# sirandreww/citizensassemblies-replication

Hardware: AMD Instinct MI355X
Metric: LEGACY panels/sec (node) at sf_e_110 shape; XtX MFMA util; speedup vs CPU (higher is better)
Workload: dtype int32/u64 (integer draw), fp4 MFMA -> exact int pairs; 1 GPU; sf_e_110: 1000000 LEGACY panels/GPU/step, k=110, n=1727, C=7, F=31, counts+pairs+unique; instance=sf_e_110, parallelism=panel shards x1, pipeline=draws on their own stream, 2 steps ahead of the counting

## Files before the change

### citizensassemblies-replication_amd/csrc/csa_legacy.hip

```cpp
#include <hip/hip_runtime.h>

#include <algorithm>
#include <type_traits>
#include <cstdlib>
#include <cstdarg>
#include <cstdio>
#include <cstring>
#include <string>
#include <vector>

#include "../../include/csa_legacy.h"

namespace {

thread_local std::string g_err;

int fail(int code, const char *fmt, ...) {
    char buf[512];
    va_list ap;
    va_start(ap, fmt);
    vsnprintf(buf, sizeof buf, fmt, ap);
    va_end(ap);
    g_err = buf;
    return code;
// ... 66 lines not shown
struct DrawArgs {
    const uint64_t *featmask;
    const int32_t *fmin, *fmax, *sel0, *rem0;
    const uint64_t *present0;
    const uint32_t *pmask;
    const int32_t *addr_next;
    int32_t n, F, W, Ws, k;
    uint32_t max_attempts, attempt_base;
    int32_t single;
    uint64_t seed, panel_begin, n_panels;
    uint64_t *panels;
    uint64_t *hashes;
    uint32_t *attempts;
    int32_t *picks;
    uint16_t *picks16;
    uint32_t *status;
    unsigned long long *stats;
    const uint64_t *panel_list;
    const unsigned long long *n_panels_dev;
    int32_t *sel_out, *rem_out;
    uint64_t *present_out;
    uint32_t *xt;
    int32_t npad;
};


template <int CTRL, int ROW_MASK = 0xF, bool BOUND_ZERO = false>
__device__ __forceinline__ int dpp(int old, int v) {
    return __builtin_amdgcn_update_dpp(old, v, CTRL, ROW_MASK, 0xF, BOUND_ZERO);
}

template <int LVL>
__device__ __forceinline__ int partner(int v) {
    if constexpr (LVL == 0) return dpp<0xB1, 0xF, true>(0, v);
    else if constexpr (LVL == 1) return dpp<0x4E, 0xF, true>(0, v);
    else if constexpr (LVL == 2) return dpp<0x141, 0xF, true>(0, v);
    else if constexpr (LVL == 3) return dpp<0x140, 0xF, true>(0, v);
    else if constexpr (LVL == 4) return __shfl_xor(v, 16);
    else return __shfl_xor(v, 32);
}

template <int LVL>
__device__ __forceinline__ uint64_t partner64(uint64_t v) {
    const uint32_t lo = (uint32_t)partner<LVL>((int)(uint32_t)v);
    const uint32_t hi = (uint32_t)partner<LVL>((int)(uint32_t)(v >> 32));
    return ((uint64_t)hi << 32) | lo;
// ... 371 lines not shown
    uint32_t k4, k2, k1;
    uint32_t r4, r2, r1;
};
__device__ __forceinline__ XtLane xt_lane_consts(int lane) {
    XtLane c;
    const bool b3 = (lane >> 3) & 1, b2 = (lane >> 2) & 1, b1 = (lane >> 1) & 1, b0 = lane & 1;
    c.s8_send = b3 ? 0x06040200u : 0x07050301u;
    c.s8_lo = b3 ? 0x03050104u : 0x05020400u;
    c.s8_hi = b3 ? 0x03070106u : 0x07020600u;
    c.k4 = b2 ? 0xF0F0F0F0u : 0x0F0F0F0Fu;
    c.k2 = b1 ? 0xCCCCCCCCu : 0x33333333u;
    c.k1 = b0 ? 0xAAAAAAAAu : 0x55555555u;
    c.r4 = b2 ? 4u : 28u;
    c.r2 = b1 ? 2u : 30u;
    c.r1 = b0 ? 1u : 31u;
    return c;
}
template <int CTRL>
__device__ __forceinline__ uint32_t xt_dpp(uint32_t v) {
    return (uint32_t)__builtin_amdgcn_update_dpp(0, (int)v, CTRL, 0xF, 0xF, true);
}
__device__ __forceinline__ uint32_t xt_merge(uint32_t x, uint32_t y, uint32_t keep, uint32_t rot) {
    const uint32_t t = __builtin_amdgcn_alignbit(y, y, rot);
    return (keep & x) | (~keep & t);
}
__device__ __forceinline__ void wave_transpose64(uint32_t &lo, uint32_t &hi, const XtLane &c) {
    {
        const auto r = __builtin_amdgcn_permlane32_swap(lo, hi, false, false);
        lo = r[0];
        hi = r[1];
    }
    {
        const uint32_t A = __builtin_amdgcn_perm(hi, lo, 0x05040100u), B = __builtin_amdgcn_perm(hi, lo, 0x07060302u);
        const auto r = __builtin_amdgcn_permlane16_swap(A, B, false, false);
        lo = __builtin_amdgcn_perm(r[1], r[0], 0x05040100u);
        hi = __builtin_amdgcn_perm(r[1], r[0], 0x07060302u);
    }
    {
        const uint32_t R = xt_dpp<0x128>(__builtin_amdgcn_perm(hi, lo, c.s8_send));
        lo = __builtin_amdgcn_perm(R, lo, c.s8_lo);
        hi = __builtin_amdgcn_perm(R, hi, c.s8_hi);
    }
    lo = xt_merge(lo, xt_dpp<0x141>(xt_dpp<0x1B>(lo)), c.k4, c.r4);
    hi = xt_merge(hi, xt_dpp<0x141>(xt_dpp<0x1B>(hi)), c.k4, c.r4);
    lo = xt_merge(lo, xt_dpp<0x4E>(lo), c.k2, c.r2);
    hi = xt_merge(hi, xt_dpp<0x4E>(hi), c.k2, c.r2);
    lo = xt_merge(lo, xt_dpp<0xB1>(lo), c.k1, c.r1);
// ... 926 lines not shown
                atomicAdd(&over_s, 1u);
        }
    }
    __syncthreads();
    for (int b = threadIdx.x; b < (int)n_bins; b += blockDim.x)
        if (h[b]) atomicAdd(hist + b, (unsigned long long)h[b]);
    if (threadIdx.x == 0 && over_s) atomicAdd(overflow, (unsigned long long)over_s);
}

}

void csa_set_last_error(const char *msg) { g_err = msg ? msg : ""; }

struct csa_instance {
    int32_t n = 0, C = 0, F = 0, W = 0, Ws = 0;
    int device = 0;
    std::vector<int32_t> pf, fmin, fmax, fcat, pool;
    std::vector<int32_t> sel0;
    std::vector<uint64_t> featmask;
    uint64_t *d_featmask = nullptr;
    int32_t *d_fmin = nullptr, *d_fmax = nullptr, *d_sel0 = nullptr, *d_rem0 = nullptr;
    uint64_t *d_present0 = nullptr;
    uint32_t *d_pmask = nullptr;
    int32_t *d_addr_next = nullptr;
    int32_t max_abs = 0;
    bool zero_max_min = false;
    bool sel_over_max = false;
    int32_t max_slack = 0;
    bool need8 = true;
    void *scratch[32] = {};
    size_t scratch_bytes[32] = {};
    hipStream_t stream = nullptr;
    hipStream_t sdraw = nullptr, spost = nullptr;
    hipEvent_t drawn = nullptr;
    uint16_t *d_picks16 = nullptr;
    size_t picks_bytes = 0;
    hipEvent_t picks_done = nullptr;
    bool picks_pending = false;
    std::vector<int32_t> rem0h, addr_h;
    std::vector<uint64_t> present0h;
    uint64_t gen = 1;
    std::vector<csa_instance *> replicas;
    std::vector<uint64_t> replica_gen;
    unsigned long long *d_stats = nullptr;
    uint64_t panels_drawn = 0;
};
// ... 152 lines not shown
        case 4: return draw_fn<G, FPL, 4, GEN>();
        case 8: if constexpr (G == 16) return draw_fn<G, FPL, 8, GEN>(); else return nullptr;
        case 16: if constexpr (G == 16) return draw_fn<G, FPL, 16, GEN>(); else return nullptr;
        default: return nullptr;
    }
}

template <int G, bool GEN>
const void *draw_fn_fw(int fpl, int wpl) {
    switch (fpl) {
        case 1: return draw_fn_w<G, 1, GEN>(wpl);
        case 2: return draw_fn_w<G, 2, GEN>(wpl);
        case 4: return draw_fn_w<G, 4, GEN>(wpl);
        default: return nullptr;
    }
}

int pow2_ceil_int(int x) {
    int p = 1;
    while (p < x) p <<= 1;
    return p;
}

int pick_draw_config(const csa_instance *I, bool general, DrawConfig &c) {
    general = general || I->d_addr_next;
    const bool reg_ok = I->F <= 32 && I->d_pmask && !I->zero_max_min && I->W <= 32 && I->max_abs < 32768 &&
                        !I->sel_over_max && I->max_slack <= 255;
    const bool lane_ok = reg_ok && I->F > 16;
    const bool wide_ok = I->F <= 64 && I->W <= 128 && !I->zero_max_min && I->max_abs < 32768 && !I->sel_over_max;
    const bool g16_ok = I->F <= 64 && I->W <= 256;
    const bool solo_ok = reg_ok && I->F <= 16;
    int choice = general ? 64 : solo_ok ? 1 : lane_ok ? 2 : wide_ok ? 8 : g16_ok ? 16 : 64;
    if (const char *e = getenv("CSA_DRAW_KERNEL")) {
        if (!general && !strcmp(e, "solo") && solo_ok) choice = 1;
        else if (!general && !strcmp(e, "lane") && lane_ok && !solo_ok) choice = 2;
        else if (!general && !strcmp(e, "wide") && wide_ok) choice = 8;
        else if (!general && !strcmp(e, "16") && g16_ok) choice = 16;
        else if (!general && !strcmp(e, "64")) choice = 64;
    }
    c.G = choice;
    if (choice == 1) {
        c.solo = true;
        c.FPL = std::max(8, pow2_ceil_int(I->F));
        c.WPL = I->W <= 4 ? 4 : I->W <= 8 ? 8 : I->W <= 16 ? 16 : I->W <= 28 ? 28 : 32;
        c.k8 = I->need8;
        c.np = c.FPL >= 16 ? slack_planes(I->max_slack) : 8;
        c.fn = solo_fn(c.FPL, c.WPL, c.k8, c.np);
        if (!c.fn) return fail(CSA_E_UNSUPPORTED, "no solo draw kernel for F=%d W=%d", I->F, I->W);
        return CSA_OK;
    }
    if (choice == 8) {
        const int fpl = (I->F + 7) / 8;
        c.wide = true;
        c.FPL = fpl <= 2 ? 2 : fpl <= 4 ? 4 : fpl <= 5 ? 5 : 8;
        c.WPL = I->W <= 32 ? 4 : I->W <= 64 ? 8 : 16;
        c.fn = wide_fn(c.FPL, c.WPL);
        if (!c.fn) return fail(CSA_E_UNSUPPORTED, "no wide draw kernel for F=%d W=%d", I->F, I->W);
        return CSA_OK;
    }
    if (choice == 2) {
        c.lane = true;
        c.FPL = std::max(8, pow2_ceil_int(I->F));
        c.WPL = I->W <= 4 ? 4 : I->W <= 8 ? 8 : I->W <= 16 ? 16 : I->W <= 28 ? 28 : 32;
        c.k8 = I->need8;
        c.np = slack_planes(I->max_slack);
        c.fn = lane_fn(c.FPL, c.WPL, c.k8, c.np);
        if (!c.fn) return fail(CSA_E_UNSUPPORTED, "no lane draw kernel for F=%d W=%d", I->F, I->W);
        return CSA_OK;
    }
    c.FPL = pow2_ceil_int((I->F + c.G - 1) / c.G);
    c.WPL = pow2_ceil_int(std::max(1, (I->W + c.G - 1) / c.G));
    if (general)
        c.fn = draw_fn_fw<64, true>(c.FPL, c.WPL);
    else
        c.fn = c.G == 16 ? draw_fn_fw<16, false>(c.FPL, c.WPL) : draw_fn_fw<64, false>(c.FPL, c.WPL);
    if (!c.fn)
        return fail(CSA_E_UNSUPPORTED, "no draw kernel for F=%d n=%d (G=%d needs FPL=%d WPL=%d)", I->F, I->n, c.G,
                    c.FPL, c.WPL);
    return CSA_OK;
}

__global__ void empty_panels_kernel(uint64_t n_panels, uint32_t *attempts, uint32_t *status, uint64_t panel_begin,
                                    int rejected) {
    const uint64_t i = (uint64_t)blockIdx.x * blockDim.x + threadIdx.x;
    if (i >= n_panels) return;
    if (rejected) {
        if (i == 0) raise_status(status, CSA_E_ATTEMPT_LIMIT, panel_begin);
    } else if (attempts) {
        attempts[i] = 1u;
    }
}

int lane_picks(csa_instance *I, uint64_t count, hipStream_t st, uint16_t **out) {
    if (!I->picks_done) HIPCHK(hipEventCreateWithFlags(&I->picks_done, hipEventDisableTiming));
    if (I->picks_pending) HIPCHK(hipStreamWaitEvent(st, I->picks_done, 0));
    const size_t bytes = std::max<uint64_t>(count, 1) * sizeof(uint16_t);
    if (I->picks_bytes < bytes) {
        if (I->picks_pending) HIPCHK(hipEventSynchronize(I->picks_done));
        if (I->d_picks16) HIPCHK(hipFree(I->d_picks16));
        I->d_picks16 = nullptr;
        I->picks_bytes = 0;
// ... 75 lines not shown
    A.W = I->W;
    A.Ws = I->Ws;
    A.k = k;
    A.max_attempts = max_attempts ? max_attempts : kDefaultMaxAttempts;
    A.attempt_base = attempt_base;
    A.single = single;
    A.seed = seed;
    A.panel_begin = panel_begin;
    A.n_panels = n_panels;
    A.panels = d_panels;
    A.hashes = d_hashes;
    A.attempts = d_attempts;
    A.picks = d_picks;
    A.picks16 = nullptr;
    A.status = d_status;
    A.stats = (single || !count_stats) ? nullptr : I->d_stats;
    A.panel_list = d_panel_list;
    A.n_panels_dev = d_list_len;
    A.sel_out = d_sel_out;
    A.rem_out = d_rem_out;
    A.present_out = d_present_out;
    A.xt = nullptr;
    A.npad = ((I->n + 255) / 256) * 256;
    if (d_picks_ext && !cfg.picks()) return fail(CSA_E_UNSUPPORTED, "this instance does not take the pick-list draw");
    csa_instance *M = const_cast<csa_instance *>(I);
    if (d_picks_ext)
        A.picks16 = d_picks_ext;
    else if (cfg.picks() && (rc = lane_picks(M, ((n_panels + 255) & ~255ull) * (uint64_t)((k + 7) & ~7), stream,
                                             &A.picks16)))
        return rc;
    const int threads = cfg.lane   ? kLaneThreads
                        : cfg.solo ? kSoloThreads
                        : cfg.wide ? kWideThreads
                                   : draw_threads(cfg.FPL, cfg.WPL);
    const int groups_wg = threads / cfg.G;
    const size_t lds = cfg.lane   ? lane_lds_bytes(cfg.FPL, cfg.WPL, I->n)
                       : cfg.solo ? solo_lds_bytes(cfg.FPL, cfg.WPL, I->n)
                       : cfg.wide ? wide_lds_bytes(cfg.G, cfg.FPL, cfg.WPL)
                                  : draw_lds_bytes(cfg.G, cfg.FPL, cfg.WPL, I->W, k, groups_wg);
    if (lds > 160 * 1024) return fail(CSA_E_UNSUPPORTED, "draw kernel needs %zu B of LDS", lds);
    static const size_t lds_pad = [] {
        const char *e = getenv("CSA_DRAW_LDS_PAD");
        return e ? (size_t)strtoull(e, nullptr, 10) : (size_t)0;
    }();
    const size_t lds_launch = (cfg.lane || cfg.solo || cfg.wide) && lds + lds_pad <= 160 * 1024 ? lds + lds_pad : lds;
    const uint64_t want = (n_panels + groups_wg - 1) / groups_wg;
// ... 228 lines not shown
    if ((rc = dalloc(&I->d_featmask, I->featmask.size())) || (rc = dalloc(&I->d_fmin, F)) ||
        (rc = dalloc(&I->d_fmax, F)) || (rc = dalloc(&I->d_sel0, F)) || (rc = dalloc(&I->d_rem0, F)) ||
        (rc = dalloc(&I->d_present0, I->W)) || (F <= 32 && (rc = dalloc(&I->d_pmask, n))) ||
        (rc = dalloc(&I->d_stats, 2))) {
        csa_instance_destroy(I);
        return rc;
    }
    std::vector<uint32_t> pmask(F <= 32 ? n : 0, 0u);
    for (int p = 0; p < (int)pmask.size(); ++p)
        for (int c = 0; c < C; ++c) pmask[p] |= 1u << person_feat[(size_t)p * C + c];
    hipError_t e = hipSuccess;
    e = e ? e : hipMemcpy(I->d_featmask, I->featmask.data(), I->featmask.size() * 8, hipMemcpyHostToDevice);
    e = e ? e : hipMemcpy(I->d_fmin, fmin, F * 4, hipMemcpyHostToDevice);
    e = e ? e : hipMemcpy(I->d_fmax, fmax, F * 4, hipMemcpyHostToDevice);
    e = e ? e : hipMemcpy(I->d_sel0, zeros.data(), F * 4, hipMemcpyHostToDevice);
    e = e ? e : hipMemcpy(I->d_rem0, I->pool.data(), F * 4, hipMemcpyHostToDevice);
    if (I->W) e = e ? e : hipMemcpy(I->d_present0, present.data(), I->W * 8, hipMemcpyHostToDevice);
    if (!pmask.empty()) e = e ? e : hipMemcpy(I->d_pmask, pmask.data(), pmask.size() * 4, hipMemcpyHostToDevice);
    e = e ? e : hipMemset(I->d_stats, 0, 16);
    if (e != hipSuccess) {
        csa_instance_destroy(I);
        return fail(CSA_E_HIP, "instance upload: %s", hipGetErrorString(e));
    }
    *out = I;
    return CSA_OK;
}

void csa_instance_destroy(csa_instance *I) {
    if (!I) return;
    ScopedDevice sd(I->device);
    if (I->picks_done && I->picks_pending) (void)hipEventSynchronize(I->picks_done);
    if (I->sdraw) (void)hipStreamSynchronize(I->sdraw);
    if (I->spost) (void)hipStreamSynchronize(I->spost);
    if (I->stream) (void)hipStreamSynchronize(I->stream);
    if (I->d_featmask) (void)hipFree(I->d_featmask);
    if (I->d_fmin) (void)hipFree(I->d_fmin);
    if (I->d_fmax) (void)hipFree(I->d_fmax);
    if (I->d_sel0) (void)hipFree(I->d_sel0);
    if (I->d_rem0) (void)hipFree(I->d_rem0);
    if (I->d_present0) (void)hipFree(I->d_present0);
    if (I->d_pmask) (void)hipFree(I->d_pmask);
    if (I->d_addr_next) (void)hipFree(I->d_addr_next);
    if (I->d_picks16) (void)hipFree(I->d_picks16);
    if (I->d_stats) (void)hipFree(I->d_stats);
    for (int i = 0; i < kScratchSlots; ++i)
        if (I->scratch[i]) (void)hipFree(I->scratch[i]);
    if (I->picks_done) (void)hipEventDestroy(I->picks_done);
    if (I->drawn) (void)hipEventDestroy(I->drawn);
    if (I->stream) (void)hipStreamDestroy(I->stream);
    if (I->sdraw) (void)hipStreamDestroy(I->sdraw);
    if (I->spost) (void)hipStreamDestroy(I->spost);
    for (csa_instance *R : I->replicas)
        if (R) csa_instance_destroy(R);
    delete I;
}

int csa_instance_draw_stats(csa_instance *I, int32_t reset, uint64_t *out) {
    if (!I || !out) return fail(CSA_E_INVALID, "draw_stats: bad arguments");
    uint64_t acc[3] = {0, 0, 0};
    std::vector<csa_instance *> all{I};
    for (csa_instance *R : I->replicas)
        if (R) all.push_back(R);
    for (csa_instance *X : all) {
        ScopedDevice sd(X->device);
// ... 57 lines not shown
    if (C) *C = I->C;
    if (F) *F = I->F;
    if (W) *W = I->W;
    return CSA_OK;
}

int csa_instance_set_state(csa_instance *I, const int32_t *sel, const int32_t *rem, const uint64_t *present) {
    if (!I) return fail(CSA_E_INVALID, "null instance");
    ScopedDevice sd(I->device);
    std::vector<int32_t> zeros(I->F, 0);
    std::vector<uint64_t> all(I->W, 0ull);
    for (int p = 0; p < I->n; ++p) all[p >> 6] |= 1ull << (p & 63);
    int32_t mx = 0;
    for (int f = 0; f < I->F; ++f) mx = std::max(mx, std::abs(I->fmin[f]));
    I->sel_over_max = false;
    I->max_slack = 0;
    for (int f = 0; f < I->F; ++f) {
        const int32_t s = sel ? sel[f] : 0;
        if (sel) mx = std::max(mx, std::abs(s));
        if (s > I->fmax[f] || (I->fmax[f] > 0 && s == I->fmax[f])) I->sel_over_max = true;
        if (I->fmax[f] > 0) I->max_slack = std::max(I->max_slack, I->fmax[f] - s);
    }
    I->max_abs = mx;
    update_need8(I);
    if (present)
        for (int w = 0; w < I->W; ++w)
            if (present[w] & ~all[w]) return fail(CSA_E_INVALID, "present mask has bits beyond n");
    HIPCHK(hipMemcpy(I->d_sel0, sel ? sel : zeros.data(), I->F * 4, hipMemcpyHostToDevice));
    I->sel0.assign(sel ? sel : zeros.data(), (sel ? sel : zeros.data()) + I->F);
    HIPCHK(hipMemcpy(I->d_rem0, rem ? rem : I->pool.data(), I->F * 4, hipMemcpyHostToDevice));
    if (I->W) HIPCHK(hipMemcpy(I->d_present0, present ? present : all.data(), I->W * 8, hipMemcpyHostToDevice));
    if (rem) I->rem0h.assign(rem, rem + I->F); else I->rem0h.clear();
    if (present) I->present0h.assign(present, present + I->W); else I->present0h.clear();
    ++I->gen;
    return CSA_OK;
}

int csa_instance_set_address(csa_instance *I, const int32_t *addr_next) {
    if (!I) return fail(CSA_E_INVALID, "null instance");
    ScopedDevice sd(I->device);
    if (I->picks_pending) HIPCHK(hipEventSynchronize(I->picks_done));
    if (!addr_next) {
        if (I->d_addr_next) HIPCHK(hipFree(I->d_addr_next));
        I->d_addr_next = nullptr;
        I->addr_h.clear();
        ++I->gen;
        return CSA_OK;
    }
    for (int p = 0; p < I->n; ++p)
        if (addr_next[p] < 0 || addr_next[p] >= I->n) return fail(CSA_E_INVALID, "addr_next[%d] out of range", p);
    if (!I->d_addr_next) {
        int rc = dalloc(&I->d_addr_next, (size_t)I->n);
        if (rc) return rc;
    }
    HIPCHK(hipMemcpy(I->d_addr_next, addr_next, (size_t)I->n * 4, hipMemcpyHostToDevice));
    I->addr_h.assign(addr_next, addr_next + I->n);
    ++I->gen;
    return CSA_OK;
// ... 918 lines not shown
```

### citizensassemblies-replication_amd/csrc/draw_lane.inc

```

constexpr int kLaneThreads = 256;
constexpr int kLaneSlots = 8;

__host__ __device__ inline size_t lane_lds_bytes(int FN, int WN, int n) {
    const size_t LS = (size_t)WN + 1;
    const size_t draw = (size_t)2 * FN * LS * 8 + 64
                        + (size_t)((n + 3) & ~3) * 4
                        + (size_t)4 * FN * 4
                        + (size_t)2 * WN * 8
                        + (size_t)(kLaneThreads / 64) * kLaneSlots * WN * 8
                        + (size_t)(kLaneThreads / 64) * kLaneSlots * FN * 4;
    const size_t pack = (size_t)(kLaneThreads / 2) * (2 * (size_t)WN + 1) * 4;
    return draw > pack ? draw : pack;
}

__device__ __forceinline__ void philox_lane(uint32_t &c0, uint32_t &c1, uint32_t &c2, uint32_t &c3, uint32_t k0,
                                            uint32_t k1) {
#pragma unroll
    for (int r = 0; r < 10; ++r) {
        if (r) {
            k0 += 0x9E3779B9u;
            k1 += 0xBB67AE85u;
        }
        asm volatile("" : "+s"(k0), "+s"(k1));
// ... 10 lines not shown
    int r;
    asm("v_bcnt_u32_b32 %0, %1, %2" : "=v"(r) : "v"(x), "v"(acc));
    return r;
}

typedef short short2_t __attribute__((ext_vector_type(2)));
__device__ __forceinline__ short2_t as_s2(int v) { return __builtin_bit_cast(short2_t, v); }
__device__ __forceinline__ int as_i(short2_t v) { return __builtin_bit_cast(int, v); }
__device__ __forceinline__ int kneed(int key) { return (int)as_s2(key).x; }
__device__ __forceinline__ int krem(int key) { return (int)as_s2(key).y; }
__device__ __forceinline__ int kpack(int need, int rem) { return (int)(((uint32_t)rem << 16) | ((uint32_t)need & 0xFFFFu)); }
__device__ __forceinline__ bool kbeats(int key, int best) {
    const short2_t a = as_s2(key), b = as_s2(best);
    return (int)a.x * (int)b.y > (int)b.x * (int)a.y;
}

#ifndef CSA_LANE_OCC
#define CSA_LANE_OCC 4
#endif

typedef signed char schar4_t __attribute__((ext_vector_type(4)));
__device__ __forceinline__ int k8need(int key) { return (int)__builtin_bit_cast(schar4_t, key).x; }
__device__ __forceinline__ int k8rem(int key) { return (int)as_s2(key).y; }
__device__ __forceinline__ int k8pack(int need, int rem, int idx) {
    return (int)(((uint32_t)rem << 16) | ((uint32_t)(idx + 1 - (need < 0)) & 0xFFu) << 8 | ((uint32_t)need & 0xFFu));
}
__device__ __forceinline__ int k8idx1(int key) { return (int)((((uint32_t)key >> 8) & 0xFFu) + (((uint32_t)key >> 7) & 1u)); }
template <bool K8>
constexpr int kDrawSentinel = K8 ? (1 << 16) | 0x009C : (1 << 16) | 0xFF9C;
__device__ __forceinline__ bool k8beats(int key, int best) {
    return k8need(key) * k8rem(best) > k8need(best) * k8rem(key);
}

#ifdef CSA_LANE_STAMPS
__device__ unsigned long long g_lane_stamps[24];
#define LANE_STAMP(k)                                              \
    do {                                                           \
        const uint64_t t_ = __builtin_amdgcn_s_memtime();          \
        st_acc[k] += t_ - st_prev;                                 \
        st_prev = t_;                                              \
    } while (0)
#define LANE_REGION(name, k, cond)                                                                \
    do {                                                                                          \
        __builtin_amdgcn_sched_barrier(0);       \
        asm volatile(";@region " #name);                                                          \
        const uint64_t b_ = __ballot(cond);                                                       \
         \
                                   \
        atomicAdd(&st_cnt[k], (uint32_t)(b_ != 0ull &&                                            \
                                         (int)(threadIdx.x & 63) == __ffsll((long long)__ballot(1)) - 1)); \
    } while (0)
#else
#define LANE_STAMP(k) \
    do {              \
    } while (0)
#define LANE_REGION(name, k, cond) \
    do {                           \
    } while (0)
#endif


constexpr int kPackRows = 128;
template <int PPW, int CH>
__device__ __forceinline__ void pack_tile_rows(const DrawArgs &A, uint32_t *tile, uint64_t pb, int rows) {
    static_assert(CH == 4 || CH == 8, "8- or 16-byte chunks");
    using unit_t = typename std::conditional<CH == 8, uint4, uint2>::type;
    const int W = A.W, k = A.k, kpad = (k + 7) & ~7, nch = kpad / CH;
    __syncthreads();
    const int R = 2 * W + 1;
    for (int t = threadIdx.x; 4 * t < kPackRows * R; t += blockDim.x) {
        if (4 * t + 3 < kPackRows * R) *reinterpret_cast<uint4 *>(tile + 4 * t) = make_uint4(0u, 0u, 0u, 0u);
        else for (int u = 4 * t; u < kPackRows * R; ++u) tile[u] = 0u;
    }
    const uint64_t wg = pb / PPW;
    const int p0 = (int)(pb % PPW);
    const unit_t *src = reinterpret_cast<const unit_t *>(A.picks16 + (wg * nch * PPW + p0) * CH);
    const int nu = nch * kPackRows;
    __syncthreads();
    constexpr int kChunks = 8;
    for (int e0 = 0; e0 < nu; e0 += kChunks * kLaneThreads) {
        unit_t v[kChunks];
#pragma unroll
        for (int u = 0; u < kChunks; ++u) {
            const int e = e0 + u * kLaneThreads + (int)threadIdx.x;
            const int r = e & (kPackRows - 1), c = e >> 7;
            if (e < nu && r < rows) v[u] = src[(uint64_t)c * PPW + r];
        }
#pragma unroll
        for (int u = 0; u < kChunks; ++u) {
            const int e = e0 + u * kLaneThreads + (int)threadIdx.x;
            const int r = e & (kPackRows - 1), c = e >> 7;
            if (e < nu && r < rows) {
                uint32_t w4[4];
                if constexpr (CH == 8) {
                    w4[0] = v[u].x; w4[1] = v[u].y; w4[2] = v[u].z; w4[3] = v[u].w;
                } else {
                    w4[0] = v[u].x; w4[1] = v[u].y; w4[2] = w4[3] = 0u;
                }
#pragma unroll
                for (int h = 0; h < CH; ++h) {
                    if (c * CH + h < k) {
                        const uint32_t q = (h & 1) ? w4[h >> 1] >> 16 : w4[h >> 1] & 0xFFFFu;
                        atomicOr(&tile[r * R + (q >> 5)], 1u << (q & 31));
                    }
                }
            }
        }
    }
    __syncthreads();
    uint64_t *dst = A.panels + pb * (uint64_t)W;
    const float rw = 1.0f / (float)W;
    for (int t = threadIdx.x; t < rows * W; t += blockDim.x) {
        const int r = min(rows - 1, (int)(((float)t + 0.5f) * rw)), w = t - r * W;
        dst[t] = (uint64_t)tile[r * R + 2 * w] | ((uint64_t)tile[r * R + 2 * w + 1] << 32);
    }
    if (A.hashes) {
        const int r = threadIdx.x >> 1, sub = threadIdx.x & 1;
        uint64_t h1 = 0, h2 = 0;
        if (r < rows)
            for (int w = sub; w < W; w += 2) {
                const uint64_t x = (uint64_t)tile[r * R + 2 * w] | ((uint64_t)tile[r * R + 2 * w + 1] << 32);
                h1 += fmix_a(x ^ ((uint64_t)w * 0x9E3779B97F4A7C15ull));
                h2 += fmix_b(x + ((uint64_t)w + 1) * 0xD6E8FEB86659FD93ull);
            }
        h1 += partner64<0>(h1);
        h2 += partner64<0>(h2);
        if (r < rows && sub == 0) {
            A.hashes[2 * (pb + r)] = h1;
            A.hashes[2 * (pb + r) + 1] = h2;
        }
    }
}

template <int NWAVES>
__device__ __forceinline__ void emit_xt_rows(const DrawArgs &A, const uint32_t *tile, uint64_t pb, int rows, int lane,
                                             int wave) {
    const XtLane tc = xt_lane_consts(lane);
    const int W = A.W, R = 2 * W + 1, nwd = A.npad / 64, nb = (rows + 63) / 64;
    const uint64_t b0 = pb / 64;
    for (int e = wave; e < nb * nwd; e += NWAVES) {
        const int blk = e / nwd, w = e - blk * nwd, r = 64 * blk + lane;
        uint32_t lo = 0u, hi = 0u;
        if (w < W && r < rows) {
            lo = tile[r * R + 2 * w];
            hi = tile[r * R + 2 * w + 1];
        }
        wave_transpose64(lo, hi, tc);
        uint32_t *x32 = A.xt + 2 * (b0 + blk) * (uint64_t)A.npad + 64 * w + lane;
        x32[0] = lo;
        x32[A.npad] = hi;
    }
}

template <int FN, int WN, int SK, int NP, bool K8>
__global__ __launch_bounds__(kLaneThreads, CSA_LANE_OCC) void draw_lane_kernel(DrawArgs A) {
    constexpr int G = 2;
    constexpr int LS = WN + 1;
    constexpr int WS = (WN + 1) / 2;
    constexpr int FPL = FN / G, WPL = WN / G;
    static_assert(FN == 32 && WN <= 32 && (WN % 2) == 0 && SK >= 1 && NP >= 1 && NP <= 8, "lane draw layout");
    extern __shared__ uint64_t smem[];
    const int F = A.F, W = A.W, n = A.n, k = A.k;
    uint64_t *fm = smem;
    uint64_t *fm_rev = fm + FN * LS + 8;
    uint32_t *pm = reinterpret_cast<uint32_t *>(fm_rev + FN * LS);
    int32_t *need0_s = reinterpret_cast<int32_t *>(pm + ((n + 3) & ~3));
    int32_t *rem0_s = need0_s + FN, *mnx_s = need0_s + 2 * FN;
    uint64_t *pres0_s = reinterpret_cast<uint64_t *>(need0_s + 4 * FN);
    uint64_t *pres0_rev = pres0_s + WN;
    uint64_t *slot_all = pres0_s + 2 * WN;
    int32_t *dec_all = reinterpret_cast<int32_t *>(slot_all + (kLaneThreads / 64) * kLaneSlots * WN);

    uint32_t live = 0;
    for (int f = 0; f < F; ++f) live |= (uint32_t)(A.fmax[f] != 0) << f;
    for (int t = threadIdx.x; t < FN * LS; t += blockDim.x) {
        const int f = t / LS, w = t - f * LS;
        const bool lf = f < F && ((live >> f) & 1u);
        fm[t] = (lf && w < W) ? A.featmask[f * A.Ws + w] : 0ull;
        const int wr = WN - 1 - w;
        fm_rev[t] = (lf && w < WN && wr < W) ? __brevll(A.featmask[f * A.Ws + wr]) : 0ull;
    }
    for (int t = threadIdx.x; t < n; t += blockDim.x) pm[t] = A.pmask[t] & live;
    for (int t = threadIdx.x; t < FN; t += blockDim.x) {
        const bool v = t < F && ((live >> t) & 1u);
        if constexpr (K8) {
            need0_s[t] = k8pack(v ? A.fmin[t] - A.sel0[t] : 0, v ? A.rem0[t] : 0, t);
        } else {
            need0_s[t] = v ? A.fmin[t] - A.sel0[t] : 0;
            rem0_s[t] = v ? A.rem0[t] : 0;
        }
    }
    for (int t = threadIdx.x; t < 16; t += blockDim.x) {
        const int h = t >> 3, bit = t & 7;
        uint32_t P = 0;
        for (int j = 0; j < FPL; ++j) {
            const int f = h * FPL + j;
            const bool v = f < F && ((live >> f) & 1u);
            const int sl = v ? A.fmax[f] - A.sel0[f] : 255;
            P |= (uint32_t)((sl >> bit) & 1) << j;
        }
        mnx_s[t] = (int32_t)P;
    }
    for (int t = threadIdx.x; t < WN; t += blockDim.x) {
        pres0_s[t] = t < W ? A.present0[t] : 0ull;
        pres0_rev[t] = WN - 1 - t < W ? __brevll(A.present0[WN - 1 - t]) : 0ull;
    }
    __syncthreads();

    const int lane = threadIdx.x & 63, wave = threadIdx.x >> 6;
    const int glane = lane & 1, gbase = lane & ~1;
    const int fbase = glane * FPL;
    const uint64_t *fmx = glane ? fm_rev : fm;
    const int poff = glane ? 64 * WN - 1 : 0, psgn = glane ? -1 : 1;
    uint64_t *slots = slot_all + (size_t)wave * kLaneSlots * WN;
    int32_t *decs = dec_all + wave * kLaneSlots * FN;
    const uint32_t key0 = (uint32_t)A.seed, key1 = (uint32_t)(A.seed >> 32);
    const uint64_t n_groups = (uint64_t)__builtin_amdgcn_readfirstlane(gridDim.x * (blockDim.x / G));
    const uint64_t *pres0_l = glane ? pres0_rev : pres0_s;
    uint64_t i = (uint64_t)blockIdx.x * (blockDim.x / G) + (threadIdx.x / G);
    bool active = i < A.n_panels;
    if (active && __hip_atomic_load(&A.status[0], __ATOMIC_RELAXED, __HIP_MEMORY_SCOPE_AGENT) != 0u) active = false;
    bool started = false;
    uint32_t a = 0;
    int s = 0;
    int key[FPL];
    uint64_t rm[WPL];
    uint32_t pacc_lo = 0u, pacc_hi = 0u;
    uint32_t sp[NP];
#pragma unroll
    for (int q = 0; q < NP; ++q) sp[q] = 0u;
// ... 410 lines not shown
```

### citizensassemblies-replication_amd/csrc/draw_solo.inc

```

constexpr int kSoloThreads = 256;
constexpr int kSoloSlots = 8;

__host__ __device__ inline size_t solo_lds_bytes(int FN, int WN, int n) {
    const size_t LS = (size_t)WN + 1;
    const size_t draw = (size_t)FN * LS * 8
                        + (size_t)((n + 3) & ~3) * 4
                        + (size_t)4 * FN * 4
                        + (size_t)WN * 8
                        + (size_t)(kSoloThreads / 64) * kSoloSlots * WN * 8
                        + (size_t)(kSoloThreads / 64) * kSoloSlots * FN * 4;
    const size_t pack = (size_t)kPackRows * (2 * (size_t)WN + 1) * 4;
    return draw > pack ? draw : pack;
}

#ifndef CSA_SOLO_OCC
#define CSA_SOLO_OCC 3
#endif
#ifndef CSA_SOLO_OCC8
#define CSA_SOLO_OCC8 4
#endif

template <int FN, int WN, int NP, bool K8>
__global__ __launch_bounds__(kSoloThreads, FN <= 8 ? CSA_SOLO_OCC8 : CSA_SOLO_OCC) void draw_solo_kernel(DrawArgs A) {
    constexpr int LS = WN + 1;
    constexpr bool kSlackPlanes = FN >= 16;
    static_assert(FN <= 32 && WN <= 32 && (FN % 8) == 0 && (WN % 2) == 0 && NP >= 1 && NP <= 8, "solo draw layout");
    extern __shared__ uint64_t smem[];
    const int F = A.F, W = A.W, n = A.n, k = A.k;
    uint64_t *fm = smem;
    uint32_t *pm = reinterpret_cast<uint32_t *>(fm + FN * LS);
    int32_t *need0_s = reinterpret_cast<int32_t *>(pm + ((n + 3) & ~3));
    int32_t *rem0_s = need0_s + FN, *mnx_s = need0_s + 2 * FN;
    uint64_t *pres0_s = reinterpret_cast<uint64_t *>(need0_s + 4 * FN);
    uint64_t *slot_all = pres0_s + WN;
    int32_t *cnt_all = reinterpret_cast<int32_t *>(slot_all + (kSoloThreads / 64) * kSoloSlots * WN);

    uint32_t live = 0;
    for (int f = 0; f < F; ++f) live |= (uint32_t)(A.fmax[f] != 0) << f;
    for (int t = threadIdx.x; t < FN * LS; t += blockDim.x) {
        const int f = t / LS, w = t - f * LS;
        const bool lf = f < F && ((live >> f) & 1u);
        fm[t] = (lf && w < W) ? A.featmask[f * A.Ws + w] : 0ull;
    }
    for (int t = threadIdx.x; t < n; t += blockDim.x) pm[t] = A.pmask[t] & live;
    for (int t = threadIdx.x; t < FN; t += blockDim.x) {
        const bool v = t < F && ((live >> t) & 1u);
        if constexpr (K8) {
            need0_s[t] = k8pack(v ? A.fmin[t] - A.sel0[t] : 0, v ? A.rem0[t] : 0, t);
        } else {
            need0_s[t] = v ? A.fmin[t] - A.sel0[t] : 0;
            rem0_s[t] = v ? A.rem0[t] : 0;
        }
    }
    if constexpr (!kSlackPlanes) {
        for (int t = threadIdx.x; t < FN; t += blockDim.x) {
            const bool v = t < F && ((live >> t) & 1u);
            mnx_s[t] = v ? A.fmin[t] - A.fmax[t] + 1 : -(1 << 30);
        }
    }
    for (int t = threadIdx.x; kSlackPlanes && t < 8; t += blockDim.x) {
        uint32_t P = 0;
        for (int j = 0; j < FN; ++j) {
            const bool v = j < F && ((live >> j) & 1u);
            const int sl = v ? A.fmax[j] - A.sel0[j] : 255;
            P |= (uint32_t)((sl >> t) & 1) << j;
        }
        mnx_s[t] = (int32_t)P;
    }
    for (int t = threadIdx.x; t < WN; t += blockDim.x) pres0_s[t] = t < W ? A.present0[t] : 0ull;
    __syncthreads();

    const int lane = threadIdx.x & 63, wave = threadIdx.x >> 6;
    uint64_t *slots = slot_all + (size_t)wave * kSoloSlots * WN;
    int32_t *cnts = cnt_all + wave * kSoloSlots * FN;
    const uint32_t key0 = (uint32_t)A.seed, key1 = (uint32_t)(A.seed >> 32);
    const uint64_t n_lanes = (uint64_t)__builtin_amdgcn_readfirstlane(gridDim.x * blockDim.x);
    uint64_t i = (uint64_t)blockIdx.x * blockDim.x + threadIdx.x;
    bool active = i < A.n_panels;
    if (active && __hip_atomic_load(&A.status[0], __ATOMIC_RELAXED, __HIP_MEMORY_SCOPE_AGENT) != 0u) active = false;
    bool started = false;
    uint32_t a = 0;
    int s = 0;
    int key[FN];
    uint64_t rm[WN];
    uint64_t pacc = 0ull;
    uint32_t sp[NP];
#pragma unroll
    for (int q = 0; q < NP; ++q) sp[q] = 0u;
    const int kpad = (k + 7) & ~7;
#pragma unroll
    for (int j = 0; j < FN; ++j) key[j] = 0;
#pragma unroll
    for (int j = 0; j < WN; ++j) rm[j] = 0ull;
// ... 320 lines not shown
```

Before: 284.0 million panels/s.

## Prebuild draw shared-memory image on host and copy it in with vector loads

Builds a host-side packed image of the per-instance draw tables (feature masks, reversed masks, pmask, need/rem keys, slack planes, presence) and uploads it once, so each lane/solo draw block fills shared memory with a bulk uint4 copy instead of computing the tables per block. It also restructures the pick-packing loop so each thread owns a row and skips per-element bounds checks on full chunks. The panel emit and xt transpose stores are changed to use incremental pointer arithmetic, and xt_merge now uses a bitop3 instruction. The image must be rebuilt whenever the start state changes, which adds host work and a device buffer per instance.

```diff
diff --git a/citizensassemblies-replication_amd/csrc/csa_legacy.hip b/citizensassemblies-replication_amd/csrc/csa_legacy.hip
--- a/citizensassemblies-replication_amd/csrc/csa_legacy.hip
+++ b/citizensassemblies-replication_amd/csrc/csa_legacy.hip
@@ -112,6 +112,7 @@
     uint64_t *present_out;
     uint32_t *xt;
     int32_t npad;
+    const uint64_t *image;
 };
 
 
@@ -529,7 +530,7 @@
 }
 __device__ __forceinline__ uint32_t xt_merge(uint32_t x, uint32_t y, uint32_t keep, uint32_t rot) {
     const uint32_t t = __builtin_amdgcn_alignbit(y, y, rot);
-    return (keep & x) | (~keep & t);
+    return __builtin_amdgcn_bitop3_b32(keep, x, t, 0xCA);
 }
 __device__ __forceinline__ void wave_transpose64(uint32_t &lo, uint32_t &hi, const XtLane &c) {
     {
@@ -1502,6 +1503,7 @@
     int32_t *d_fmin = nullptr, *d_fmax = nullptr, *d_sel0 = nullptr, *d_rem0 = nullptr;
     uint64_t *d_present0 = nullptr;
     uint32_t *d_pmask = nullptr;
+    uint64_t *d_image = nullptr;
     int32_t *d_addr_next = nullptr;
     int32_t max_abs = 0;
     bool zero_max_min = false;
@@ -1700,6 +1702,14 @@
     return p;
 }
 
+bool reg_kernel_shape(const csa_instance *I, bool &lane, int &fn, int &wn) {
+    if (I->F > 32 || I->W > 32 || !I->d_pmask) return false;
+    lane = I->F > 16;
+    fn = std::max(8, pow2_ceil_int(I->F));
+    wn = I->W <= 4 ? 4 : I->W <= 8 ? 8 : I->W <= 16 ? 16 : I->W <= 28 ? 28 : 32;
+    return true;
+}
+
 int pick_draw_config(const csa_instance *I, bool general, DrawConfig &c) {
     general = general || I->d_addr_next;
     const bool reg_ok = I->F <= 32 && I->d_pmask && !I->zero_max_min && I->W <= 32 && I->max_abs < 32768 &&
@@ -1719,8 +1729,8 @@
     c.G = choice;
     if (choice == 1) {
         c.solo = true;
-        c.FPL = std::max(8, pow2_ceil_int(I->F));
-        c.WPL = I->W <= 4 ? 4 : I->W <= 8 ? 8 : I->W <= 16 ? 16 : I->W <= 28 ? 28 : 32;
+        bool lane_shape;
+        reg_kernel_shape(I, lane_shape, c.FPL, c.WPL);
         c.k8 = I->need8;
         c.np = c.FPL >= 16 ? slack_planes(I->max_slack) : 8;
         c.fn = solo_fn(c.FPL, c.WPL, c.k8, c.np);
@@ -1738,8 +1748,8 @@
     }
     if (choice == 2) {
         c.lane = true;
-        c.FPL = std::max(8, pow2_ceil_int(I->F));
-        c.WPL = I->W <= 4 ? 4 : I->W <= 8 ? 8 : I->W <= 16 ? 16 : I->W <= 28 ? 28 : 32;
+        bool lane_shape;
+        reg_kernel_shape(I, lane_shape, c.FPL, c.WPL);
         c.k8 = I->need8;
         c.np = slack_planes(I->max_slack);
         c.fn = lane_fn(c.FPL, c.WPL, c.k8, c.np);
@@ -1755,6 +1765,81 @@
     if (!c.fn)
         return fail(CSA_E_UNSUPPORTED, "no draw kernel for F=%d n=%d (G=%d needs FPL=%d WPL=%d)", I->F, I->n, c.G,
                     c.FPL, c.WPL);
+    return CSA_OK;
+}
+
+int draw_image_build(csa_instance *I) {
+    bool lane = false;
+    int FN = 0, WN = 0;
+    if (!reg_kernel_shape(I, lane, FN, WN)) return CSA_OK;
+    const int F = I->F, W = I->W, n = I->n, LS = WN + 1;
+    const DrawImage L = draw_image_layout(lane, FN, WN, n);
+    std::vector<uint32_t> img((size_t)2 * L.words, 0u);
+    auto put64 = [&](int word, uint64_t v) {
+        img[2 * (size_t)word] = (uint32_t)v;
+        img[2 * (size_t)word + 1] = (uint32_t)(v >> 32);
+    };
+    auto brev64 = [](uint64_t x) {
+        uint64_t r = 0;
+        for (int b = 0; b < 64; ++b) r |= ((x >> b) & 1ull) << (63 - b);
+        return r;
+    };
+    uint32_t live = 0;
+    for (int f = 0; f < F; ++f) live |= (uint32_t)(I->fmax[f] != 0) << f;
+    auto alive = [&](int f) { return f < F && ((live >> f) & 1u); };
+    for (int f = 0; f < F; ++f) {
+        if (!alive(f)) continue;
+        const uint64_t *row = I->featmask.data() + (size_t)f * I->Ws;
+        for (int w = 0; w < W; ++w) put64(f * LS + w, row[w]);
+        for (int t = 0; lane && t < WN; ++t)
+            if (WN - 1 - t < W) put64(L.fm_rev + f * LS + t, brev64(row[WN - 1 - t]));
+    }
+    for (int p = 0; p < n; ++p) {
+        uint32_t m = 0;
+        for (int c = 0; c < I->C; ++c) m |= 1u << I->pf[(size_t)p * I->C + c];
+        img[2 * (size_t)L.pm + p] = m & live;
+    }
+    uint32_t *need0 = img.data() + 2 * (size_t)L.need0, *rem0 = need0 + FN, *mnx = need0 + 2 * FN;
+    const int32_t *rem = I->rem0h.empty() ? I->pool.data() : I->rem0h.data();
+    for (int t = 0; t < FN; ++t) {
+        const int need = alive(t) ? I->fmin[t] - I->sel0[t] : 0, rm = alive(t) ? rem[t] : 0;
+        if (I->need8) {
+            need0[t] = (uint32_t)k8pack(need, rm, t);
+        } else {
+            need0[t] = (uint32_t)need;
+            rem0[t] = (uint32_t)rm;
+        }
+    }
+    if (FN >= 16) {
+        const int halves = lane ? 2 : 1, FPL = FN / halves;
+        for (int h = 0; h < halves; ++h)
+            for (int bit = 0; bit < 8; ++bit) {
+                uint32_t P = 0;
+                for (int j = 0; j < FPL; ++j) {
+                    const int f = h * FPL + j;
+                    const int sl = alive(f) ? I->fmax[f] - I->sel0[f] : 255;
+                    P |= (uint32_t)((sl >> bit) & 1) << j;
+                }
+                mnx[8 * h + bit] = P;
+            }
+    } else {
+        for (int t = 0; t < FN; ++t) mnx[t] = (uint32_t)(alive(t) ? I->fmin[t] - I->fmax[t] + 1 : -(1 << 30));
+    }
+    for (int t = 0; t < WN; ++t) {
+        auto pres = [&](int w) -> uint64_t {
+            if (w >= W) return 0ull;
+            if (!I->present0h.empty()) return I->present0h[w];
+            return w < n / 64 ? ~0ull : (1ull << (n & 63)) - 1ull;
+        };
+        put64(L.pres0 + t, pres(t));
+        if (lane) put64(L.pres0_rev + t, brev64(pres(WN - 1 - t)));
+    }
+    ScopedDevice sd(I->device);
+    if (!I->d_image) {
+        int rc = dalloc(&I->d_image, (size_t)L.words);
+        if (rc) return rc;
+    }
+    HIPCHK(hipMemcpy(I->d_image, img.data(), (size_t)L.words * 8, hipMemcpyHostToDevice));
     return CSA_OK;
 }
 
@@ -1876,6 +1961,8 @@
     A.present_out = d_present_out;
     A.xt = nullptr;
     A.npad = ((I->n + 255) / 256) * 256;
+    A.image = I->d_image;
+    if ((cfg.lane || cfg.solo) && !A.image) return fail(CSA_E_INVALID, "the instance has no draw image");
     if (d_picks_ext && !cfg.picks()) return fail(CSA_E_UNSUPPORTED, "this instance does not take the pick-list draw");
     csa_instance *M = const_cast<csa_instance *>(I);
     if (d_picks_ext)
@@ -2150,6 +2237,10 @@
         csa_instance_destroy(I);
         return fail(CSA_E_HIP, "instance upload: %s", hipGetErrorString(e));
     }
+    if ((rc = draw_image_build(I))) {
+        csa_instance_destroy(I);
+        return rc;
+    }
     *out = I;
     return CSA_OK;
 }
@@ -2168,6 +2259,7 @@
     if (I->d_rem0) (void)hipFree(I->d_rem0);
     if (I->d_present0) (void)hipFree(I->d_present0);
     if (I->d_pmask) (void)hipFree(I->d_pmask);
+    if (I->d_image) (void)hipFree(I->d_image);
     if (I->d_addr_next) (void)hipFree(I->d_addr_next);
     if (I->d_picks16) (void)hipFree(I->d_picks16);
     if (I->d_stats) (void)hipFree(I->d_stats);
@@ -2271,18 +2363,18 @@
         if (I->fmax[f] > 0) I->max_slack = std::max(I->max_slack, I->fmax[f] - s);
     }
     I->max_abs = mx;
-    update_need8(I);
     if (present)
         for (int w = 0; w < I->W; ++w)
             if (present[w] & ~all[w]) return fail(CSA_E_INVALID, "present mask has bits beyond n");
     HIPCHK(hipMemcpy(I->d_sel0, sel ? sel : zeros.data(), I->F * 4, hipMemcpyHostToDevice));
     I->sel0.assign(sel ? sel : zeros.data(), (sel ? sel : zeros.data()) + I->F);
+    update_need8(I);
     HIPCHK(hipMemcpy(I->d_rem0, rem ? rem : I->pool.data(), I->F * 4, hipMemcpyHostToDevice));
     if (I->W) HIPCHK(hipMemcpy(I->d_present0, present ? present : all.data(), I->W * 8, hipMemcpyHostToDevice));
     if (rem) I->rem0h.assign(rem, rem + I->F); else I->rem0h.clear();
     if (present) I->present0h.assign(present, present + I->W); else I->present0h.clear();
     ++I->gen;
-    return CSA_OK;
+    return draw_image_build(I);
 }
 
 int csa_instance_set_address(csa_instance *I, const int32_t *addr_next) {
diff --git a/citizensassemblies-replication_amd/csrc/draw_lane.inc b/citizensassemblies-replication_amd/csrc/draw_lane.inc
--- a/citizensassemblies-replication_amd/csrc/draw_lane.inc
+++ b/citizensassemblies-replication_amd/csrc/draw_lane.inc
@@ -56,7 +56,7 @@
 typedef signed char schar4_t __attribute__((ext_vector_type(4)));
 __device__ __forceinline__ int k8need(int key) { return (int)__builtin_bit_cast(schar4_t, key).x; }
 __device__ __forceinline__ int k8rem(int key) { return (int)as_s2(key).y; }
-__device__ __forceinline__ int k8pack(int need, int rem, int idx) {
+__host__ __device__ inline int k8pack(int need, int rem, int idx) {
     return (int)(((uint32_t)rem << 16) | ((uint32_t)(idx + 1 - (need < 0)) & 0xFFu) << 8 | ((uint32_t)need & 0xFFu));
 }
 __device__ __forceinline__ int k8idx1(int key) { return (int)((((uint32_t)key >> 8) & 0xFFu) + (((uint32_t)key >> 7) & 1u)); }
@@ -93,6 +93,42 @@
     } while (0)
 #endif
 
+struct DrawImage {
+    int fm_rev, pm, need0, pres0, pres0_rev, words;
+};
+__host__ __device__ constexpr DrawImage draw_image_layout(bool lane, int FN, int WN, int n) {
+    DrawImage L = {};
+    L.fm_rev = FN * (WN + 1) + 8;
+    L.pm = lane ? L.fm_rev + FN * (WN + 1) : FN * (WN + 1);
+    L.need0 = L.pm + ((n + 3) & ~3) / 2;
+    L.pres0 = L.need0 + 2 * FN;
+    L.pres0_rev = L.pres0 + WN;
+    L.words = L.pres0 + (lane ? 2 : 1) * WN;
+    return L;
+}
+__device__ __forceinline__ void load_draw_image(uint64_t *smem, const uint64_t *image, int n16) {
+    constexpr int B = 4, T = 256;
+    const uint4 *src = reinterpret_cast<const uint4 *>(image) + threadIdx.x;
+    uint4 *dst = reinterpret_cast<uint4 *>(smem) + threadIdx.x;
+    int base = 0;
+    for (; base + B * T <= n16; base += B * T) {
+        uint4 v[B];
+#pragma unroll
+        for (int u = 0; u < B; ++u) v[u] = src[base + u * T];
+#pragma unroll
+        for (int u = 0; u < B; ++u) dst[base + u * T] = v[u];
+    }
+    const int left = n16 - base - (int)threadIdx.x;
+    const uint4 *img = reinterpret_cast<const uint4 *>(image);
+    uint4 v[B];
+#pragma unroll
+    for (int u = 0; u < B; ++u) v[u] = img[min(base + u * T + (int)threadIdx.x, n16 - 1)];
+#pragma unroll
+    for (int u = 0; u < B; ++u)
+        if (u * T < left) dst[base + u * T] = v[u];
+    __syncthreads();
+}
+
 
 constexpr int kPackRows = 128;
 template <int PPW, int CH>
@@ -109,33 +145,45 @@
     const uint64_t wg = pb / PPW;
     const int p0 = (int)(pb % PPW);
     const unit_t *src = reinterpret_cast<const unit_t *>(A.picks16 + (wg * nch * PPW + p0) * CH);
-    const int nu = nch * kPackRows;
     __syncthreads();
-    constexpr int kChunks = 8;
-    for (int e0 = 0; e0 < nu; e0 += kChunks * kLaneThreads) {
-        unit_t v[kChunks];
-#pragma unroll
-        for (int u = 0; u < kChunks; ++u) {
-            const int e = e0 + u * kLaneThreads + (int)threadIdx.x;
-            const int r = e & (kPackRows - 1), c = e >> 7;
-            if (e < nu && r < rows) v[u] = src[(uint64_t)c * PPW + r];
-        }
-#pragma unroll
-        for (int u = 0; u < kChunks; ++u) {
-            const int e = e0 + u * kLaneThreads + (int)threadIdx.x;
-            const int r = e & (kPackRows - 1), c = e >> 7;
-            if (e < nu && r < rows) {
-                uint32_t w4[4];
-                if constexpr (CH == 8) {
-                    w4[0] = v[u].x; w4[1] = v[u].y; w4[2] = v[u].z; w4[3] = v[u].w;
-                } else {
-                    w4[0] = v[u].x; w4[1] = v[u].y; w4[2] = w4[3] = 0u;
-                }
-#pragma unroll
-                for (int h = 0; h < CH; ++h) {
-                    if (c * CH + h < k) {
-                        const uint32_t q = (h & 1) ? w4[h >> 1] >> 16 : w4[h >> 1] & 0xFFFFu;
-                        atomicOr(&tile[r * R + (q >> 5)], 1u << (q & 31));
+    constexpr int kChunks = 8, kRowSets = kLaneThreads / kPackRows;
+    static_assert(kPackRows % 64 == 0 && kLaneThreads % kPackRows == 0, "a wave's threads share their chunk index");
+    const int r = (int)(threadIdx.x & (kPackRows - 1));
+    const int cfirst = __builtin_amdgcn_readfirstlane((int)(threadIdx.x / kPackRows));
+    if (r < rows) {
+        uint32_t *trow = tile + r * R;
+        const unit_t *srow = src + r;
+        for (int c0 = cfirst; c0 < nch; c0 += kRowSets * kChunks) {
+            unit_t v[kChunks];
+#pragma unroll
+            for (int u = 0; u < kChunks; ++u) {
+                const int c = c0 + kRowSets * u;
+                if (c < nch) v[u] = srow[(uint64_t)c * PPW];
+            }
+#pragma unroll
+            for (int u = 0; u < kChunks; ++u) {
+                const int c = c0 + kRowSets * u;
+                if (c < nch) {
+                    uint32_t w4[4];
+                    if constexpr (CH == 8) {
+                        w4[0] = v[u].x; w4[1] = v[u].y; w4[2] = v[u].z; w4[3] = v[u].w;
+                    } else {
+                        w4[0] = v[u].x; w4[1] = v[u].y; w4[2] = w4[3] = 0u;
+                    }
+                    if ((c + 1) * CH <= k) {
+#pragma unroll
+                        for (int h = 0; h < CH; ++h) {
+                            const uint32_t q = (h & 1) ? w4[h >> 1] >> 16 : w4[h >> 1] & 0xFFFFu;
+                            atomicOr(&trow[q >> 5], 1u << (q & 31));
+                        }
+                    } else {
+#pragma unroll
+                        for (int h = 0; h < CH; ++h) {
+                            if (c * CH + h < k) {
+                                const uint32_t q = (h & 1) ? w4[h >> 1] >> 16 : w4[h >> 1] & 0xFFFFu;
+                                atomicOr(&trow[q >> 5], 1u << (q & 31));
+                            }
+                        }
                     }
                 }
             }
@@ -143,10 +191,21 @@
     }
     __syncthreads();
     uint64_t *dst = A.panels + pb * (uint64_t)W;
-    const float rw = 1.0f / (float)W;
-    for (int t = threadIdx.x; t < rows * W; t += blockDim.x) {
-        const int r = min(rows - 1, (int)(((float)t + 0.5f) * rw)), w = t - r * W;
-        dst[t] = (uint64_t)tile[r * R + 2 * w] | ((uint64_t)tile[r * R + 2 * w + 1] << 32);
+    {
+        const int nt = rows * W, dq = kLaneThreads / W, dm = kLaneThreads - dq * W, step = dq * R + 2 * dm;
+        int t = (int)threadIdx.x;
+        const int r0 = (int)(((float)t + 0.5f) * (1.0f / (float)W));
+        int w = t - r0 * W;
+        const uint32_t *tp = tile + r0 * R + 2 * w;
+        for (; t < nt; t += kLaneThreads) {
+            dst[t] = (uint64_t)tp[0] | ((uint64_t)tp[1] << 32);
+            w += dm;
+            tp += step;
+            if (w >= W) {
+                w -= W;
+                tp += 1;
+            }
+        }
     }
     if (A.hashes) {
         const int r = threadIdx.x >> 1, sub = threadIdx.x & 1;
@@ -170,19 +229,23 @@
 __device__ __forceinline__ void emit_xt_rows(const DrawArgs &A, const uint32_t *tile, uint64_t pb, int rows, int lane,
                                              int wave) {
     const XtLane tc = xt_lane_consts(lane);
-    const int W = A.W, R = 2 * W + 1, nwd = A.npad / 64, nb = (rows + 63) / 64;
-    const uint64_t b0 = pb / 64;
-    for (int e = wave; e < nb * nwd; e += NWAVES) {
-        const int blk = e / nwd, w = e - blk * nwd, r = 64 * blk + lane;
-        uint32_t lo = 0u, hi = 0u;
-        if (w < W && r < rows) {
-            lo = tile[r * R + 2 * w];
-            hi = tile[r * R + 2 * w + 1];
-        }
-        wave_transpose64(lo, hi, tc);
-        uint32_t *x32 = A.xt + 2 * (b0 + blk) * (uint64_t)A.npad + 64 * w + lane;
-        x32[0] = lo;
-        x32[A.npad] = hi;
+    const int W = A.W, R = 2 * W + 1, npad = A.npad, nwd = npad / 64, nb = (rows + 63) / 64;
+    const int w0 = __builtin_amdgcn_readfirstlane(wave);
+    for (int blk = 0; blk < nb; ++blk) {
+        const uint32_t *trow = tile + (64 * blk + lane) * R + 2 * w0;
+        char *xlo = reinterpret_cast<char *>(A.xt + 2 * (pb / 64 + blk) * (uint64_t)npad), *xhi = xlo + 4 * (size_t)npad;
+        uint32_t off = 4u * (uint32_t)(64 * w0 + lane);
+        int w = w0;
+        for (; w < W; w += NWAVES, trow += 2 * NWAVES, off += 256u * NWAVES) {
+            uint32_t lo = trow[0], hi = trow[1];
+            wave_transpose64(lo, hi, tc);
+            *reinterpret_cast<uint32_t *>(xlo + off) = lo;
+            *reinterpret_cast<uint32_t *>(xhi + off) = hi;
+        }
+        for (; w < nwd; w += NWAVES, off += 256u * NWAVES) {
+            *reinterpret_cast<uint32_t *>(xlo + off) = 0u;
+            *reinterpret_cast<uint32_t *>(xhi + off) = 0u;
+        }
     }
 }
 
@@ -194,52 +257,19 @@
     constexpr int FPL = FN / G, WPL = WN / G;
     static_assert(FN == 32 && WN <= 32 && (WN % 2) == 0 && SK >= 1 && NP >= 1 && NP <= 8, "lane draw layout");
     extern __shared__ uint64_t smem[];
-    const int F = A.F, W = A.W, n = A.n, k = A.k;
+    const int n = A.n, k = A.k;
+    const DrawImage L = draw_image_layout(true, FN, WN, n);
     uint64_t *fm = smem;
-    uint64_t *fm_rev = fm + FN * LS + 8;
-    uint32_t *pm = reinterpret_cast<uint32_t *>(fm_rev + FN * LS);
-    int32_t *need0_s = reinterpret_cast<int32_t *>(pm + ((n + 3) & ~3));
+    uint64_t *fm_rev = fm + L.fm_rev;
+    uint32_t *pm = reinterpret_cast<uint32_t *>(fm + L.pm);
+    int32_t *need0_s = reinterpret_cast<int32_t *>(fm + L.need0);
     int32_t *rem0_s = need0_s + FN, *mnx_s = need0_s + 2 * FN;
-    uint64_t *pres0_s = reinterpret_cast<uint64_t *>(need0_s + 4 * FN);
-    uint64_t *pres0_rev = pres0_s + WN;
-    uint64_t *slot_all = pres0_s + 2 * WN;
+    uint64_t *pres0_s = fm + L.pres0;
+    uint64_t *pres0_rev = fm + L.pres0_rev;
+    uint64_t *slot_all = fm + L.words;
     int32_t *dec_all = reinterpret_cast<int32_t *>(slot_all + (kLaneThreads / 64) * kLaneSlots * WN);
 
-    uint32_t live = 0;
-    for (int f = 0; f < F; ++f) live |= (uint32_t)(A.fmax[f] != 0) << f;
-    for (int t = threadIdx.x; t < FN * LS; t += blockDim.x) {
-        const int f = t / LS, w = t - f * LS;
-        const bool lf = f < F && ((live >> f) & 1u);
-        fm[t] = (lf && w < W) ? A.featmask[f * A.Ws + w] : 0ull;
-        const int wr = WN - 1 - w;
-        fm_rev[t] = (lf && w < WN && wr < W) ? __brevll(A.featmask[f * A.Ws + wr]) : 0ull;
-    }
-    for (int t = threadIdx.x; t < n; t += blockDim.x) pm[t] = A.pmask[t] & live;
-    for (int t = threadIdx.x; t < FN; t += blockDim.x) {
-        const bool v = t < F && ((live >> t) & 1u);
-        if constexpr (K8) {
-            need0_s[t] = k8pack(v ? A.fmin[t] - A.sel0[t] : 0, v ? A.rem0[t] : 0, t);
-        } else {
-            need0_s[t] = v ? A.fmin[t] - A.sel0[t] : 0;
-            rem0_s[t] = v ? A.rem0[t] : 0;
-        }
-    }
-    for (int t = threadIdx.x; t < 16; t += blockDim.x) {
-        const int h = t >> 3, bit = t & 7;
-        uint32_t P = 0;
-        for (int j = 0; j < FPL; ++j) {
-            const int f = h * FPL + j;
-            const bool v = f < F && ((live >> f) & 1u);
-            const int sl = v ? A.fmax[f] - A.sel0[f] : 255;
-            P |= (uint32_t)((sl >> bit) & 1) << j;
-        }
-        mnx_s[t] = (int32_t)P;
-    }
-    for (int t = threadIdx.x; t < WN; t += blockDim.x) {
-        pres0_s[t] = t < W ? A.present0[t] : 0ull;
-        pres0_rev[t] = WN - 1 - t < W ? __brevll(A.present0[WN - 1 - t]) : 0ull;
-    }
-    __syncthreads();
+    load_draw_image(smem, A.image, L.words / 2);
 
     const int lane = threadIdx.x & 63, wave = threadIdx.x >> 6;
     const int glane = lane & 1, gbase = lane & ~1;
diff --git a/citizensassemblies-replication_amd/csrc/draw_solo.inc b/citizensassemblies-replication_amd/csrc/draw_solo.inc
--- a/citizensassemblies-replication_amd/csrc/draw_solo.inc
+++ b/citizensassemblies-replication_amd/csrc/draw_solo.inc
@@ -27,49 +27,17 @@
     constexpr bool kSlackPlanes = FN >= 16;
     static_assert(FN <= 32 && WN <= 32 && (FN % 8) == 0 && (WN % 2) == 0 && NP >= 1 && NP <= 8, "solo draw layout");
     extern __shared__ uint64_t smem[];
-    const int F = A.F, W = A.W, n = A.n, k = A.k;
+    const int n = A.n, k = A.k;
+    const DrawImage L = draw_image_layout(false, FN, WN, n);
     uint64_t *fm = smem;
-    uint32_t *pm = reinterpret_cast<uint32_t *>(fm + FN * LS);
-    int32_t *need0_s = reinterpret_cast<int32_t *>(pm + ((n + 3) & ~3));
+    uint32_t *pm = reinterpret_cast<uint32_t *>(fm + L.pm);
+    int32_t *need0_s = reinterpret_cast<int32_t *>(fm + L.need0);
     int32_t *rem0_s = need0_s + FN, *mnx_s = need0_s + 2 * FN;
-    uint64_t *pres0_s = reinterpret_cast<uint64_t *>(need0_s + 4 * FN);
-    uint64_t *slot_all = pres0_s + WN;
+    uint64_t *pres0_s = fm + L.pres0;
+    uint64_t *slot_all = fm + L.words;
     int32_t *cnt_all = reinterpret_cast<int32_t *>(slot_all + (kSoloThreads / 64) * kSoloSlots * WN);
 
-    uint32_t live = 0;
-    for (int f = 0; f < F; ++f) live |= (uint32_t)(A.fmax[f] != 0) << f;
-    for (int t = threadIdx.x; t < FN * LS; t += blockDim.x) {
-        const int f = t / LS, w = t - f * LS;
-        const bool lf = f < F && ((live >> f) & 1u);
-        fm[t] = (lf && w < W) ? A.featmask[f * A.Ws + w] : 0ull;
-    }
-    for (int t = threadIdx.x; t < n; t += blockDim.x) pm[t] = A.pmask[t] & live;
-    for (int t = threadIdx.x; t < FN; t += blockDim.x) {
-        const bool v = t < F && ((live >> t) & 1u);
-        if constexpr (K8) {
-            need0_s[t] = k8pack(v ? A.fmin[t] - A.sel0[t] : 0, v ? A.rem0[t] : 0, t);
-        } else {
-            need0_s[t] = v ? A.fmin[t] - A.sel0[t] : 0;
-            rem0_s[t] = v ? A.rem0[t] : 0;
-        }
-    }
-    if constexpr (!kSlackPlanes) {
-        for (int t = threadIdx.x; t < FN; t += blockDim.x) {
-            const bool v = t < F && ((live >> t) & 1u);
-            mnx_s[t] = v ? A.fmin[t] - A.fmax[t] + 1 : -(1 << 30);
-        }
-    }
-    for (int t = threadIdx.x; kSlackPlanes && t < 8; t += blockDim.x) {
-        uint32_t P = 0;
-        for (int j = 0; j < FN; ++j) {
-            const bool v = j < F && ((live >> j) & 1u);
-            const int sl = v ? A.fmax[j] - A.sel0[j] : 255;
-            P |= (uint32_t)((sl >> t) & 1) << j;
-        }
-        mnx_s[t] = (int32_t)P;
-    }
-    for (int t = threadIdx.x; t < WN; t += blockDim.x) pres0_s[t] = t < W ? A.present0[t] : 0ull;
-    __syncthreads();
+    load_draw_image(smem, A.image, L.words / 2);
 
     const int lane = threadIdx.x & 63, wave = threadIdx.x >> 6;
     uint64_t *slots = slot_all + (size_t)wave * kSoloSlots * WN;
```

New measurement: 289.1 million panels/s (median of 6 runs). +1.8%, better.
